# alanross/AlvaAR

Measured on NVIDIA H100. Metric: frames_per_sec_720p_1000orb_20kf_ba, higher is better.
Workload: dtype u8/f64

## Files before the change

alvaar_b200/csrc/ba.cu:

```cuda
#include "alva_common.cuh"
#include "../../include/alva_b200.h"
#include <math.h>
#include <float.h>
#include <string.h>

namespace {

constexpr int NMAX = 128;
constexpr int LIN_THREADS = 128;
constexpr int NBMAX = NMAX / 6;
constexpr int MAXKEYS = NBMAX * (NBMAX + 1) / 2;
constexpr int BS_THREADS = 128;

struct BaState {
    double radius, decrease_factor, x_cost, cand_cost, xnorm, gmax, model_change;
    double se_min, se_cur, se_ref, se_cand, se_acc_ref, se_acc_cand;
    double initial_cost, push_cost;
    int reuse_diagonal, invalid_steps, iteration, last_success, n_success, n_iter, term, done;
    int relin, step_ok, ncols, chol_ok;
    int use_gather, nb, nbad, has_last;
    int skipped, pad0;
};

struct BaProblem {
    const double* calib;
    double* poses;
    const uint8_t* pose_const;
    double* invd;
    const int32_t* anch_kf;
    const double* anch_uv;
    const int32_t* obs_kf;
    const int32_t* obs_lm;
    const double* obs_uv;
    double *res, *Ja, *Jd;
    double *wp;
    double *nf, *gf, *scf, *diagf, *Df;
    double *ne, *ge, *sce, *diage, *De;
    double *ete, *etb, *wa, *ye;
    double *S, *rhs, *yf;
    double *cand_poses, *cand_invd;
    double *cost_part;
    int32_t *pose_col;
    int32_t *lm_start, *lm_obs;
    double* Wt;
    double* mc_part;
    double* ga_part;
    int32_t* ga_ticket;
    int32_t *obs_col, *anch_col;
    int32_t *pstart;
    uint32_t *plist;
    int32_t *blk_start;
    int32_t *blk_off;
    uint64_t *pairs;
    const int32_t* obs_lm_in;
    int32_t* obs_lm_w;
    int32_t* flags;
    double *last_poses, *last_invd;
    BaState* st;
};

struct BaDims { int nkf, nlm, nobs, nblk; double huber; int max_iter; int nlm_pad; int ecap; int nbs; int pass; };

__device__ __forceinline__ void quat_to_R(const double* q, double* R) {
    const double n = sqrt(q[0] * q[0] + q[1] * q[1] + q[2] * q[2] + q[3] * q[3]);
    const double x = q[0] / n, y = q[1] / n, z = q[2] / n, w = q[3] / n;
    const double tx = 2 * x, ty = 2 * y, tz = 2 * z;
    const double twx = tx * w, twy = ty * w, twz = tz * w, txx = tx * x, txy = ty * x, txz = tz * x;
    const double tyy = ty * y, tyz = tz * y, tzz = tz * z;
    R[0] = 1 - (tyy + tzz); R[1] = txy - twz;       R[2] = txz + twy;
    R[3] = txy + twz;       R[4] = 1 - (txx + tzz); R[5] = tyz - twx;
    R[6] = txz - twy;       R[7] = tyz + twx;       R[8] = 1 - (txx + tyy);
}

__device__ void se3_plus(const double* x, const double* delta, double* out) {
    const double* ups = delta;
    const double* om = delta + 3;
    const double theta_sq = om[0] * om[0] + om[1] * om[1] + om[2] * om[2];
    const double eps = 1e-10;
    double theta, imag, real;
    if (theta_sq < eps * eps) {
        theta = 0;
        const double t4 = theta_sq * theta_sq;
        imag = 0.5 - (1.0 / 48.0) * theta_sq + (1.0 / 3840.0) * t4;
        real = 1.0 - (1.0 / 8.0) * theta_sq + (1.0 / 384.0) * t4;
    } else {
        theta = sqrt(theta_sq);
        const double half = 0.5 * theta;
        imag = sin(half) / theta;
        real = cos(half);
    }
    const double dq[4] = {imag * om[0], imag * om[1], imag * om[2], real};
    double Rd[9];
    quat_to_R(dq, Rd);
    const double O[9] = {0, -om[2], om[1], om[2], 0, -om[0], -om[1], om[0], 0};
    double V[9];
    if (theta < eps) {
        for (int i = 0; i < 9; i++) V[i] = Rd[i];
    } else {
        const double a = (1 - cos(theta)) / theta_sq, b = (theta - sin(theta)) / (theta_sq * theta);
        for (int i = 0; i < 3; i++)
            for (int j = 0; j < 3; j++) {
                double o2 = 0;
                for (int k = 0; k < 3; k++) o2 += O[3 * i + k] * O[3 * k + j];
                V[3 * i + j] = (i == j ? 1.0 : 0.0) + a * O[3 * i + j] + b * o2;
            }
    }
    for (int i = 0; i < 3; i++)
        out[i] = V[3 * i] * ups[0] + V[3 * i + 1] * ups[1] + V[3 * i + 2] * ups[2] + Rd[3 * i] * x[0] + Rd[3 * i + 1] * x[1] +
                 Rd[3 * i + 2] * x[2];
    const double qn = sqrt(x[3] * x[3] + x[4] * x[4] + x[5] * x[5] + x[6] * x[6]);
    const double bx = x[3] / qn, by = x[4] / qn, bz = x[5] / qn, bw = x[6] / qn;
    const double ax = dq[0], ay = dq[1], az = dq[2], aw = dq[3];
    double q[4] = {aw * bx + ax * bw + ay * bz - az * by, aw * by + ay * bw + az * bx - ax * bz,
                   aw * bz + az * bw + ax * by - ay * bx, aw * bw - ax * bx - ay * by - az * bz};
    const double n = sqrt(q[0] * q[0] + q[1] * q[1] + q[2] * q[2] + q[3] * q[3]);
    for (int i = 0; i < 4; i++) out[3 + i] = q[i] / n;
}

__device__ __forceinline__ bool ba_evaluate(const double* calib, const double* anch, const double* pose, double invd, double u,
                                            double v, double ua, double va, double* res, double* Ja, double* Jp, double* Jd) {
    const double fx = calib[0], fy = calib[1], cx = calib[2], cy = calib[3];
    double Rwa[9], Rwc[9];
    quat_to_R(anch + 3, Rwa);
    quat_to_R(pose + 3, Rwc);
    const double zanch = 1.0 / invd;
    const double ap[3] = {zanch * (ua - cx) / fx, zanch * (va - cy) / fy, zanch};
    double Ra[3], wpt[3];
    for (int i = 0; i < 3; i++) {
        Ra[i] = Rwa[3 * i] * ap[0] + Rwa[3 * i + 1] * ap[1] + Rwa[3 * i + 2] * ap[2];
        wpt[i] = Ra[i] + anch[i];
    }
    const double d[3] = {wpt[0] - pose[0], wpt[1] - pose[1], wpt[2] - pose[2]};
    double cp[3];
    for (int i = 0; i < 3; i++) cp[i] = Rwc[i] * d[0] + Rwc[3 + i] * d[1] + Rwc[6 + i] * d[2];
    const double iz = 1.0 / cp[2];
// ... 151 lines not shown
            if (P.obs_col[o] >= 0) { key = P.obs_col[o] / 6; val = ((uint32_t)l << 8) | (uint32_t)(i - P.lm_start[l] + 1); }
        }
    };
    int maxobs = 0;
    for (int l = tid; l < D.nlm; l += NT) maxobs = max(maxobs, P.lm_start[l + 1] - P.lm_start[l]);
    for (int t = tid; t < nitems; t += NT) {
        int key; uint32_t val;
        item(t, key, val);
        if (key >= 0) atomicAdd(&pl_base[key + 1], 1);
    }
    __syncthreads();
    if (tid == 0) {
        P.pstart[0] = 0;
        for (int k = 0; k < NBMAX; k++) { P.pstart[k + 1] = pl_base[k + 1]; pl_base[k + 1] += pl_base[k]; }
    }
    __syncthreads();
    for (int t0 = 0; t0 < nitems; t0 += NT) {
        for (int i = tid; i < 32 * (NBMAX + 1); i += NT) (&wcount[0][0])[i] = 0;
        __syncthreads();
        int key; uint32_t val;
        item(t0 + tid, key, val);
        const uint32_t m = __match_any_sync(0xffffffffu, key);
        const int rank = __popc(m & ((1u << lane) - 1));
        if (key >= 0 && rank == 0) wcount[warp][key] = __popc(m);
        __syncthreads();
        if (tid < NBMAX) {
            int acc = 0;
            for (int wv = 0; wv < 32; wv++) { const int c = wcount[wv][tid]; wcount[wv][tid] = acc; acc += c; }
            scan_s[tid] = acc;
        }
        __syncthreads();
        if (key >= 0) P.plist[pl_base[key] + run[key] + wcount[warp][key] + rank] = val;
        __syncthreads();
        if (tid < NBMAX) run[tid] += scan_s[tid];
        __syncthreads();
    }
    maxobs = max(maxobs, __shfl_xor_sync(0xffffffffu, maxobs, 16)); maxobs = max(maxobs, __shfl_xor_sync(0xffffffffu, maxobs, 8));
    maxobs = max(maxobs, __shfl_xor_sync(0xffffffffu, maxobs, 4)); maxobs = max(maxobs, __shfl_xor_sync(0xffffffffu, maxobs, 2));
    maxobs = max(maxobs, __shfl_xor_sync(0xffffffffu, maxobs, 1));
    if (lane == 0) scan_s[warp] = maxobs;
    __syncthreads();
    if (tid == 0) {
        int mo = 0;
        for (int i = 0; i < NT / 32; i++) mo = max(mo, scan_s[i]);
        P.st->use_gather = (mo < 255 && D.nlm < 65536 && D.nobs < 65535) ? 1 : 0;
    }
}

template <bool FULL>
__device__ __forceinline__ double lin_obs(const BaProblem& P, const BaDims& D, int o, int l, const double* poses, double invd_l) {
    const int ka = P.anch_kf[l], kp = P.obs_kf[o];
    double r[2], Ja[12], Jp[12], Jd[2];
    ba_evaluate(P.calib, poses + 7 * ka, poses + 7 * kp, invd_l, P.obs_uv[2 * o], P.obs_uv[2 * o + 1], P.anch_uv[2 * l],
                P.anch_uv[2 * l + 1], r, FULL ? Ja : nullptr, Jp, Jd);
    double rho0, rho1;
    huber(r[0] * r[0] + r[1] * r[1], D.huber, rho0, rho1);
    if (FULL) {
        const double sc = sqrt(rho1);
        r[0] *= sc; r[1] *= sc;
        P.res[2 * o] = r[0]; P.res[2 * o + 1] = r[1];
        Jd[0] *= sc; Jd[1] *= sc;
        P.Jd[2 * o] = Jd[0]; P.Jd[2 * o + 1] = Jd[1];
#pragma unroll
        for (int i = 0; i < 12; i++) { Ja[i] *= sc; P.Ja[12 * o + i] = Ja[i]; }
    }
    return 0.5 * rho0;
}

template <bool FULL>
__global__ void __launch_bounds__(LIN_THREADS, 7) ba_linearize_kernel(const BaProblem* __restrict__ probs, BaDims D) {
    const BaProblem P = probs[blockIdx.y];
    __shared__ double red[LIN_THREADS];
    const BaState& st = *P.st;
    const bool active = FULL ? (st.relin && !st.done) : !st.done;
    if (!active) return;
    const int o = blockIdx.x * LIN_THREADS + threadIdx.x;
    double cost = 0;
    const int l = o < D.nobs ? P.obs_lm[o] : -1;
    if (l >= 0) cost = lin_obs<FULL>(P, D, o, l, FULL ? P.poses : P.cand_poses, (FULL ? P.invd : P.cand_invd)[l]);
    const double tot = block_sum<LIN_THREADS>(cost, red);
    if (threadIdx.x == 0) P.cost_part[blockIdx.x] = tot;
}

__device__ __forceinline__ void stats_landmark(const BaProblem& P, int l) {
    double ne = 0, ge = 0;
    for (int i = P.lm_start[l]; i < P.lm_start[l + 1]; i++) {
        const int o = P.lm_obs[i];
        const double d0 = P.Jd[2 * o], d1 = P.Jd[2 * o + 1];
        ne += d0 * d0 + d1 * d1;
        ge += d0 * P.res[2 * o] + d1 * P.res[2 * o + 1];
    }
    P.ne[l] = ne;
    P.ge[l] = ge;
}
__device__ __forceinline__ void stats_pose_partial(const BaProblem& P, int b, int gt, double* v) {
    int eb = 0;
    for (int i = 0; i < b; i++) eb += P.pstart[i + 1];
    const int ee = eb + P.pstart[b + 1];
#pragma unroll
    for (int i = 0; i < 12; i++) v[i] = 0;
    for (int idx = eb + gt; idx < ee; idx += BS_THREADS) {
        const uint32_t en = P.plist[idx];
        const int l = en >> 8, su = en & 0xff;
        const int ob = P.lm_start[l];
        if (su) {
            const int o = P.lm_obs[ob + su - 1];
            const double r0 = P.res[2 * o], r1 = P.res[2 * o + 1];
#pragma unroll
            for (int c = 0; c < 6; c++) {
                const double j0 = -P.Ja[12 * o + c], j1 = -P.Ja[12 * o + 6 + c];
                v[c] += j0 * j0 + j1 * j1;
                v[6 + c] += j0 * r0 + j1 * r1;
            }
        } else {
            for (int i = ob; i < P.lm_start[l + 1]; i++) {
                const int o = P.lm_obs[i];
                const double r0 = P.res[2 * o], r1 = P.res[2 * o + 1];
#pragma unroll
                for (int c = 0; c < 6; c++) {
                    const double j0 = P.Ja[12 * o + c], j1 = P.Ja[12 * o + 6 + c];
                    v[c] += j0 * j0 + j1 * j1;
                    v[6 + c] += j0 * r0 + j1 * r1;
                }
            }
        }
    }
}

__global__ void __launch_bounds__(BS_THREADS) ba_stats_kernel(const BaProblem* __restrict__ probs, BaDims D) {
    const BaProblem P = probs[blockIdx.y];
    const BaState& st = *P.st;
    if (st.done || !st.relin) return;
    __shared__ double part[4][12];
    if ((int)blockIdx.x < D.nbs) {
        const int l = blockIdx.x * BS_THREADS + threadIdx.x;
        if (l >= D.nlm) return;
        stats_landmark(P, l);
        return;
    }
    const int b = blockIdx.x - D.nbs;
    if (b >= st.ncols / 6) return;
    const int lane = threadIdx.x & 31, warp = threadIdx.x >> 5;
    double v[12];
    stats_pose_partial(P, b, threadIdx.x, v);
#pragma unroll
    for (int i = 0; i < 12; i++) {
#pragma unroll
        for (int off = 16; off; off >>= 1) v[i] += __shfl_xor_sync(0xffffffffu, v[i], off);
        if (lane == 0) part[warp][i] = v[i];
    }
    __syncthreads();
    if (threadIdx.x < 12) {
        const double t = part[0][threadIdx.x] + part[1][threadIdx.x] + part[2][threadIdx.x] + part[3][threadIdx.x];
        if (threadIdx.x < 6) P.nf[6 * b + threadIdx.x] = t;
        else P.gf[6 * b + threadIdx.x - 6] = t;
    }
}

template <int MODE>
__global__ void __launch_bounds__(32) ba_pairs_kernel(const BaProblem* __restrict__ probs, BaDims D) {
    const BaProblem P = probs[blockIdx.y];
    BaState& st = *P.st;
    const int nb = st.ncols / 6, bi = blockIdx.x, lane = threadIdx.x;
    if (!st.use_gather) return;
    __shared__ int cnt[NBMAX];
    __shared__ int boff[NBMAX];
    if (bi >= nb) {
        if (MODE == 0) for (int bj = lane; bj < NBMAX; bj += 32) P.blk_start[bi * NBMAX + bj + 1] = 0;
        return;
    }
    int base_row = 0;
    if (MODE == 1) {
        int sum = 0;
        for (int i = lane; i < bi * NBMAX; i += 32) sum += P.blk_start[i + 1];
#pragma unroll
        for (int off = 16; off; off >>= 1) sum += __shfl_xor_sync(0xffffffffu, sum, off);
        base_row = sum;
    }
    if (lane < NBMAX) cnt[lane] = 0;
    if (lane == 0) {
        int run = base_row;
        for (int bj = 0; bj < NBMAX; bj++) {
            boff[bj] = run;
            if (MODE == 1) { P.blk_off[bi * NBMAX + bj] = run; run += P.blk_start[bi * NBMAX + bj + 1]; }
        }
    }
    __syncwarp();
    int eb = 0;
    for (int i = 0; i < bi; i++) eb += P.pstart[i + 1];
    const int ee = eb + P.pstart[bi + 1];
    for (int c0 = eb; c0 < ee; c0 += 32) {
        const int idx = c0 + lane;
        const bool live = idx < ee;
        const uint32_t en = live ? P.plist[idx] : 0u;
        const int l = en >> 8, su = en & 0xff;
        const int ob = live ? P.lm_start[l] : 0, ns = live ? P.lm_start[l + 1] - ob : -1;
        int cv0 = -1, cv1 = -1, cv2 = -1, cv3 = -1, o1 = -1, o2 = -1, o3 = -1, ou = 0xffff;
        if (live) {
            cv0 = P.anch_col[l];
            o1 = ns >= 1 ? P.lm_obs[ob] : -1; o2 = ns >= 2 ? P.lm_obs[ob + 1] : -1; o3 = ns >= 3 ? P.lm_obs[ob + 2] : -1;
            if (o1 >= 0) cv1 = P.obs_col[o1];
            if (o2 >= 0) cv2 = P.obs_col[o2];
            if (o3 >= 0) cv3 = P.obs_col[o3];
            if (MODE == 1 && su) ou = su == 1 ? o1 : su == 2 ? o2 : su == 3 ? o3 : P.lm_obs[ob + su - 1];
        }
        for (int sv = 0; sv <= 255; sv++) {
            if (!__any_sync(0xffffffffu, live && sv <= ns)) break;
            int bjv = -1, bjv_ov = 0xffff;
            if (live && sv <= ns) {
                const int ov = sv == 0 ? 0xffff : sv == 1 ? o1 : sv == 2 ? o2 : sv == 3 ? o3 : P.lm_obs[ob + sv - 1];
                bjv_ov = ov;
                const int cv = sv == 0 ? cv0 : sv == 1 ? cv1 : sv == 2 ? cv2 : sv == 3 ? cv3 : P.obs_col[ov];
                if (cv >= 0) { const int bj = cv / 6; if (bj > bi || (bj == bi && sv >= su)) bjv = bj; }
                if (MODE == 0 && cv >= 0 && cv / 6 == bi && sv > su) st.use_gather = 0;
            }
            const uint32_t m = __match_any_sync(0xffffffffu, bjv);
            if (bjv >= 0) {
                const int rank = __popc(m & ((1u << lane) - 1));
                const int old = cnt[bjv];
                if (MODE == 1) {
                    const int pos = boff[bjv] + old + rank;
                    if (pos < D.ecap)
                        P.pairs[pos] = ((uint64_t)l << 48) | ((uint64_t)su << 40) | ((uint64_t)sv << 32) | ((uint64_t)(ou & 0xffff) << 16) |
                                       (uint64_t)(bjv_ov & 0xffff);
                }
                __syncwarp(m);
                if (rank == 0) cnt[bjv] = old + __popc(m);
            }
            __syncwarp();
        }
    }
    if (MODE == 0) {
        if (lane < NBMAX) P.blk_start[bi * NBMAX + lane + 1] = cnt[lane];
    } else if (bi == nb - 1 && lane == 0) {
        int total = base_row;
        for (int bj = 0; bj < NBMAX; bj++) total += cnt[bj];
        if (total > D.ecap) st.use_gather = 0;
    }
}

constexpr int CT_THREADS = 1024;
__device__ void ba_pre_body(const BaProblem& P, const BaDims& D) {
    BaState& st = *P.st;
    __shared__ double red[34];
    __shared__ int go;
    const int tid = threadIdx.x, NT = blockDim.x;
    const int n = st.ncols;
    if (st.done) return;
    if (st.relin) {
        double c = 0;
        for (int i = tid; i < D.nblk; i += NT) c += P.cost_part[i];
        const double x_cost = block_sum_dyn(c, red);
        double xn = 0;
        for (int k = tid; k < D.nkf; k += NT)
            if (P.pose_col[k] >= 0) for (int i = 0; i < 7; i++) xn += P.poses[7 * k + i] * P.poses[7 * k + i];
        for (int l = tid; l < D.nlm; l += NT)
            if (P.lm_start[l + 1] > P.lm_start[l]) xn += P.invd[l] * P.invd[l];
        xn = block_sum_dyn(xn, red);
        double gm = 0;
        for (int k = tid; k < D.nkf; k += NT) {
            const int c0 = P.pose_col[k];
            if (c0 < 0) continue;
            double dlt[6], out[7];
            for (int i = 0; i < 6; i++) dlt[i] = -P.gf[c0 + i];
            se3_plus(P.poses + 7 * k, dlt, out);
            for (int i = 0; i < 7; i++) gm = fmax(gm, fabs(P.poses[7 * k + i] - out[i]));
        }
        for (int l = tid; l < D.nlm; l += NT)
            if (P.lm_start[l + 1] > P.lm_start[l]) gm = fmax(gm, fabs(P.ge[l]));
        gm = block_max_dyn(gm, red);
        if (st.iteration == 0) {
            for (int i = tid; i < n; i += NT) P.scf[i] = 1.0 / (1.0 + sqrt(P.nf[i]));
            for (int l = tid; l < D.nlm; l += NT) P.sce[l] = 1.0 / (1.0 + sqrt(P.ne[l]));
        }
        __syncthreads();
        if (tid == 0) {
            st.x_cost = x_cost; st.xnorm = sqrt(xn); st.gmax = gm; st.push_cost = x_cost;
            if (st.iteration == 0) {
                st.initial_cost = x_cost;
                st.se_min = st.se_cur = st.se_ref = st.se_cand = x_cost;
            }
            st.relin = 0;
        }
    }
    __syncthreads();
    if (tid == 0) {
        if (st.last_success) st.n_success++;
        st.n_iter++;
        int cont = 1;
        if (st.iteration >= D.max_iter) { st.term = 1; cont = 0; }
        else if (st.last_success && st.gmax <= 1e-10) { st.term = 0; cont = 0; }
        else if (st.radius <= 1e-32) { st.term = 0; cont = 0; }
        if (!cont) st.done = 1;
        else { st.iteration++; st.last_success = 0; }
        go = cont;
    }
    __syncthreads();
    if (!go) return;
    const bool reuse = st.reuse_diagonal;
    const double radius = st.radius;
    __syncthreads();
    for (int i = tid; i < n; i += NT) {
        if (!reuse) P.diagf[i] = fmin(fmax(P.nf[i] * P.scf[i] * P.scf[i], 1e-6), 1e32);
        P.Df[i] = sqrt(P.diagf[i] / radius);
    }
    for (int l = tid; l < D.nlm; l += NT) {
        if (!reuse) P.diage[l] = fmin(fmax(P.ne[l] * P.sce[l] * P.sce[l], 1e-6), 1e32);
        P.De[l] = sqrt(P.diage[l] / radius);
    }
    for (int i = tid; i < NMAX * NMAX; i += NT) P.S[i] = 0;
    for (int i = tid; i < NMAX; i += NT) P.rhs[i] = 0;
    __syncthreads();
    for (int i = tid; i < n; i += NT) P.S[i * NMAX + i] = P.Df[i] * P.Df[i];
    if (tid == 0) st.reuse_diagonal = 1;
}

__global__ void __launch_bounds__(CT_THREADS) ba_pre_kernel(const BaProblem* __restrict__ probs, BaDims D) {
    const BaProblem P = probs[blockIdx.x];
    ba_pre_body(P, D);
}

template <bool DENSE>
__device__ void schur_landmark(const BaProblem& P, const BaDims& D, int l) {
    if (DENSE) {
        double* row = P.Wt + (size_t)l * NMAX;
        for (int i = 0; i < NMAX; i++) row[i] = 0.0;
    }
    if (l >= D.nlm) return;
    const int b = P.lm_start[l], e = P.lm_start[l + 1];
    if (e == b) return;
    const int ca = P.pose_col[P.anch_kf[l]];
    const double sce = P.sce[l];
    double ete = P.De[l] * P.De[l], etb = 0, wa[6] = {0, 0, 0, 0, 0, 0};
    double sca[6];
    for (int c = 0; c < 6; c++) sca[c] = ca >= 0 ? P.scf[ca + c] : 0.0;
    double Saa[36];
    for (int i = 0; i < 36; i++) Saa[i] = 0;
    double rha[6] = {0, 0, 0, 0, 0, 0};
    for (int i = b; i < e; i++) {
        const int o = P.lm_obs[i];
        const int cp = P.pose_col[P.obs_kf[o]];
        const double e0 = P.Jd[2 * o] * sce, e1 = P.Jd[2 * o + 1] * sce;
        const double r0 = P.res[2 * o], r1 = P.res[2 * o + 1];
        ete += e0 * e0 + e1 * e1;
        etb += e0 * r0 + e1 * r1;
        double Fa[12], Fp[12];
        for (int c = 0; c < 6; c++) {
            Fa[c] = P.Ja[12 * o + c] * sca[c]; Fa[6 + c] = P.Ja[12 * o + 6 + c] * sca[c];
            const double s = cp >= 0 ? P.scf[cp + c] : 0.0;
            Fp[c] = -P.Ja[12 * o + c] * s; Fp[6 + c] = -P.Ja[12 * o + 6 + c] * s;
        }
        for (int c = 0; c < 6; c++) {
            wa[c] += e0 * Fa[c] + e1 * Fa[6 + c];
            P.wp[6 * o + c] = e0 * Fp[c] + e1 * Fp[6 + c];
            rha[c] += Fa[c] * r0 + Fa[6 + c] * r1;
        }
        if (ca >= 0)
            for (int a = 0; a < 6; a++)
                for (int c = 0; c < 6; c++) Saa[6 * a + c] += Fa[a] * Fa[c] + Fa[6 + a] * Fa[6 + c];
        if (cp >= 0) {
            for (int a = 0; a < 6; a++) {
                atomicAdd(&P.rhs[cp + a], Fp[a] * r0 + Fp[6 + a] * r1);
                for (int c = 0; c < 6; c++) {
                    atomicAdd(&P.S[(cp + a) * NMAX + cp + c], Fp[a] * Fp[c] + Fp[6 + a] * Fp[6 + c]);
                    if (ca >= 0) {
                        const double x = Fa[a] * Fp[c] + Fa[6 + a] * Fp[6 + c];
                        atomicAdd(&P.S[(ca + a) * NMAX + cp + c], x);
                        atomicAdd(&P.S[(cp + c) * NMAX + ca + a], x);
                    }
                }
            }
        }
    }
    const double inv = 1.0 / ete;
    P.ete[l] = ete;
    P.etb[l] = etb;
    for (int c = 0; c < 6; c++) P.wa[6 * l + c] = wa[c];
    if (ca >= 0)
        for (int a = 0; a < 6; a++) {
            atomicAdd(&P.rhs[ca + a], rha[a] - wa[a] * inv * etb);
            for (int c = 0; c < 6; c++)
                atomicAdd(&P.S[(ca + a) * NMAX + ca + c], DENSE ? Saa[6 * a + c] : Saa[6 * a + c] - wa[a] * inv * wa[c]);
        }
    if (DENSE) {
        const double rs = sqrt(inv);
        double* row = P.Wt + (size_t)l * NMAX;
        if (ca >= 0) for (int c = 0; c < 6; c++) row[ca + c] += wa[c] * rs;
        for (int i = b; i < e; i++) {
            const int oi = P.lm_obs[i];
            const int ci = P.pose_col[P.obs_kf[oi]];
            if (ci < 0) continue;
// ... 10 lines not shown
        if (ci < 0) continue;
        double wi[6];
        for (int c = 0; c < 6; c++) wi[c] = P.wp[6 * oi + c];
        for (int a = 0; a < 6; a++) atomicAdd(&P.rhs[ci + a], -wi[a] * inv * etb);
        if (ca >= 0)
            for (int a = 0; a < 6; a++)
                for (int c = 0; c < 6; c++) {
                    const double x = -wa[a] * inv * wi[c];
                    atomicAdd(&P.S[(ca + a) * NMAX + ci + c], x);
                    atomicAdd(&P.S[(ci + c) * NMAX + ca + a], x);
                }
        for (int j = b; j < e; j++) {
            const int oj = P.lm_obs[j];
            const int cj = P.pose_col[P.obs_kf[oj]];
            if (cj < 0) continue;
            for (int a = 0; a < 6; a++)
                for (int c = 0; c < 6; c++) atomicAdd(&P.S[(ci + a) * NMAX + cj + c], -wi[a] * inv * P.wp[6 * oj + c]);
        }
    }
}

template <bool DENSE>
__global__ void __launch_bounds__(128) ba_schur_kernel(const BaProblem* __restrict__ probs, BaDims D) {
    const BaProblem P = probs[blockIdx.y];
    if (P.st->done) return;
    if (!DENSE && P.st->use_gather) return;
    const int l = blockIdx.x * 128 + threadIdx.x;
    if (l >= D.nlm_pad) return;
    schur_landmark<DENSE>(P, D, l);
}

__device__ __forceinline__ void dmma_m8n8k4(double& c0, double& c1, double a, double b) {
    asm volatile("mma.sync.aligned.m8n8k4.row.col.f64.f64.f64.f64 {%0, %1}, {%2}, {%3}, {%0, %1};"
                 : "+d"(c0), "+d"(c1)
                 : "d"(a), "d"(b));
}

constexpr int SYRK_KSPLIT = 8;

__global__ void __launch_bounds__(128) ba_syrk_dmma_kernel(const BaProblem* __restrict__ probs, BaDims D) {
    const BaProblem P = probs[blockIdx.z];
    if (P.st->done) return;
    __shared__ double part[4][32][33];
    const int lane = threadIdx.x & 31, warp = threadIdx.x >> 5;
    const int bi = blockIdx.x >> 2, bj = blockIdx.x & 3;
    const int i0 = bi * 32, j0 = bj * 32;
    const int n = P.st->ncols;
    if (i0 >= n || j0 >= n) return;
    const int ksteps = D.nlm_pad / 4;
    const int per = (ksteps + SYRK_KSPLIT - 1) / SYRK_KSPLIT;
    const int kb = blockIdx.y * per, ke = min(ksteps, kb + per);
    double acc[4][4][2];
#pragma unroll
    for (int a = 0; a < 4; a++)
#pragma unroll
        for (int b = 0; b < 4; b++) acc[a][b][0] = acc[a][b][1] = 0.0;
    const int kr = lane & 3, cc = lane >> 2;
    for (int ks = kb + warp; ks < ke; ks += 4) {
        const double* row = P.Wt + (size_t)(4 * ks + kr) * NMAX;
        double av[4], bv[4];
#pragma unroll
        for (int t = 0; t < 4; t++) { av[t] = __ldg(row + i0 + 8 * t + cc); bv[t] = __ldg(row + j0 + 8 * t + cc); }
#pragma unroll
        for (int a = 0; a < 4; a++)
#pragma unroll
            for (int b = 0; b < 4; b++) dmma_m8n8k4(acc[a][b][0], acc[a][b][1], av[a], bv[b]);
    }
#pragma unroll
    for (int a = 0; a < 4; a++)
#pragma unroll
        for (int b = 0; b < 4; b++) {
            part[warp][8 * a + cc][8 * b + 2 * kr] = acc[a][b][0];
            part[warp][8 * a + cc][8 * b + 2 * kr + 1] = acc[a][b][1];
        }
    __syncthreads();
    for (int t = threadIdx.x; t < 32 * 32; t += 128) {
        const int r = t >> 5, c = t & 31;
        const double v = part[0][r][c] + part[1][r][c] + part[2][r][c] + part[3][r][c];
        if (v != 0.0) atomicAdd(&P.S[(i0 + r) * NMAX + j0 + c], -v);
    }
}


__device__ __forceinline__ void lm_landmark(const BaProblem& P, int l) {
    const int b = P.lm_start[l], e = P.lm_start[l + 1];
    if (e == b) return;
    const int ca = P.pose_col[P.anch_kf[l]];
    const double sce = P.sce[l];
    double ete = P.De[l] * P.De[l], etb = 0, wa[6] = {0, 0, 0, 0, 0, 0};
    for (int i = b; i < e; i++) {
        const int o = P.lm_obs[i];
        const int cp = P.pose_col[P.obs_kf[o]];
        const double e0 = P.Jd[2 * o] * sce, e1 = P.Jd[2 * o + 1] * sce;
        ete += e0 * e0 + e1 * e1;
        etb += e0 * P.res[2 * o] + e1 * P.res[2 * o + 1];
        for (int c = 0; c < 6; c++) {
            if (ca >= 0) wa[c] += (e0 * P.Ja[12 * o + c] + e1 * P.Ja[12 * o + 6 + c]) * P.scf[ca + c];
            P.wp[6 * o + c] = cp >= 0 ? (e0 * -P.Ja[12 * o + c] + e1 * -P.Ja[12 * o + 6 + c]) * P.scf[cp + c] : 0.0;
        }
    }
    P.ete[l] = ete;
    P.etb[l] = etb;
    for (int c = 0; c < 6; c++) P.wa[6 * l + c] = wa[c];
}
__global__ void __launch_bounds__(128) ba_lm_kernel(const BaProblem* __restrict__ probs, BaDims D) {
    const BaProblem P = probs[blockIdx.y];
    if (P.st->done) return;
    const int l = blockIdx.x * 128 + threadIdx.x;
    if (P.st->use_gather) { if (l < D.nlm) lm_landmark(P, l); }
    else if (l < D.nlm) schur_landmark<false>(P, D, l);
}

template <bool TRANSPOSE>
__device__ __forceinline__ void gather_entry(const BaProblem& P, uint64_t en, const double* sci, const double* scj, double* acc,
                                             double* rh) {
    const int l = (int)(en >> 48), su = (int)(en >> 40) & 0xff, sv = (int)(en >> 32) & 0xff;
    const double inv = 1.0 / P.ete[l], etb = P.etb[l];
    const int ou = su ? (int)(en >> 16) & 0xffff : -1, ov = sv ? (int)en & 0xffff : -1;
    double wu[6], wv[6];
#pragma unroll
    for (int c = 0; c < 6; c++) {
        wu[c] = (su ? P.wp[6 * ou + c] : P.wa[6 * l + c]) * inv;
        wv[c] = sv ? P.wp[6 * ov + c] : P.wa[6 * l + c];
    }
#define ACC(a, c) acc[TRANSPOSE ? 6 * (c) + (a) : 6 * (a) + (c)]
#pragma unroll
    for (int a = 0; a < 6; a++)
#pragma unroll
        for (int c = 0; c < 6; c++) ACC(a, c) -= wu[a] * wv[c];
    if (su == 0 && sv == 0) {
        const int ob = P.lm_start[l], oe = P.lm_start[l + 1];
        for (int i = ob; i < oe; i++) {
            const int o = P.lm_obs[i];
            double F0[6], F1[6];
#pragma unroll
            for (int c = 0; c < 6; c++) { F0[c] = P.Ja[12 * o + c] * sci[c]; F1[c] = P.Ja[12 * o + 6 + c] * sci[c]; }
            const double r0 = P.res[2 * o], r1 = P.res[2 * o + 1];
#pragma unroll
            for (int a = 0; a < 6; a++) {
                if (!TRANSPOSE) rh[a] += F0[a] * r0 + F1[a] * r1;
#pragma unroll
                for (int c = 0; c < 6; c++) ACC(a, c) += F0[a] * F0[c] + F1[a] * F1[c];
            }
        }
        if (!TRANSPOSE)
#pragma unroll
            for (int a = 0; a < 6; a++) rh[a] -= wu[a] * etb;
    } else if (su == sv) {
        double F0[6], F1[6];
#pragma unroll
        for (int c = 0; c < 6; c++) { F0[c] = -P.Ja[12 * ou + c] * sci[c]; F1[c] = -P.Ja[12 * ou + 6 + c] * sci[c]; }
        const double r0 = P.res[2 * ou], r1 = P.res[2 * ou + 1];
#pragma unroll
        for (int a = 0; a < 6; a++) {
            if (!TRANSPOSE) rh[a] += F0[a] * r0 + F1[a] * r1 - wu[a] * etb;
#pragma unroll
            for (int c = 0; c < 6; c++) ACC(a, c) += F0[a] * F0[c] + F1[a] * F1[c];
        }
    } else if (su == 0 || sv == 0) {
        const int o = su ? ou : ov;
        double A0[6], A1[6];
#pragma unroll
        for (int a = 0; a < 6; a++) {
            A0[a] = (su ? -P.Ja[12 * o + a] : P.Ja[12 * o + a]) * sci[a];
            A1[a] = (su ? -P.Ja[12 * o + 6 + a] : P.Ja[12 * o + 6 + a]) * sci[a];
        }
#pragma unroll
        for (int c = 0; c < 6; c++) {
            const double b0 = (sv ? -P.Ja[12 * o + c] : P.Ja[12 * o + c]) * scj[c];
            const double b1 = (sv ? -P.Ja[12 * o + 6 + c] : P.Ja[12 * o + 6 + c]) * scj[c];
#pragma unroll
            for (int a = 0; a < 6; a++) ACC(a, c) += A0[a] * b0 + A1[a] * b1;
        }
    }
#undef ACC
}

constexpr int GA_THREADS = 64, GA_SPLIT = 8;
constexpr int GA_GRID = NBMAX * GA_SPLIT + (MAXKEYS - NBMAX);
__global__ void __launch_bounds__(GA_THREADS, 8) ba_gather_kernel(const BaProblem* __restrict__ probs, BaDims D) {
    const BaProblem P = probs[blockIdx.y];
    const BaState& st = *P.st;
    if (st.done || !st.use_gather) return;
    int bi, bj, part = 0, nparts = 1;
    if ((int)blockIdx.x < NBMAX * GA_SPLIT) { bi = bj = blockIdx.x / GA_SPLIT; part = blockIdx.x % GA_SPLIT; nparts = GA_SPLIT; }
    else {
        int rem = blockIdx.x - NBMAX * GA_SPLIT;
        bi = 0;
        while (bi < NBMAX - 1 && rem >= NBMAX - 1 - bi) { rem -= NBMAX - 1 - bi; bi++; }
        bj = bi + 1 + rem;
    }
    if (bi >= st.nb || bj >= st.nb) return;
// ... 332 lines not shown
__global__ void ba_linearize_dump_kernel(const double* calib, const double* poses, const double* invd, const int32_t* anch_kf,
                                         const double* anch_uv, const int32_t* obs_kf, const int32_t* obs_lm,
                                         const double* obs_uv, int nobs, double hub, double* res, double* Ja, double* Jp,
                                         double* Jd, double* cost) {
    const int o = blockIdx.x * blockDim.x + threadIdx.x;
    if (o >= nobs) return;
    const int l = obs_lm[o];
    double r[2] = {0, 0}, A[12], Pp[12], Dd[2];
    for (int i = 0; i < 12; i++) A[i] = Pp[i] = 0;
    Dd[0] = Dd[1] = 0;
    double c = 0;
    if (l >= 0) {
        ba_evaluate(calib, poses + 7 * anch_kf[l], poses + 7 * obs_kf[o], invd[l], obs_uv[2 * o], obs_uv[2 * o + 1],
                    anch_uv[2 * l], anch_uv[2 * l + 1], r, A, Pp, Dd);
        double rho0, rho1;
        huber(r[0] * r[0] + r[1] * r[1], hub, rho0, rho1);
        c = 0.5 * rho0;
        const double sc = sqrt(rho1);
        r[0] *= sc; r[1] *= sc; Dd[0] *= sc; Dd[1] *= sc;
        for (int i = 0; i < 12; i++) { A[i] *= sc; Pp[i] *= sc; }
    }
    res[2 * o] = r[0]; res[2 * o + 1] = r[1]; Jd[2 * o] = Dd[0]; Jd[2 * o + 1] = Dd[1];
    for (int i = 0; i < 12; i++) { Ja[12 * o + i] = A[i]; Jp[12 * o + i] = Pp[i]; }
    cost[o] = c;
}

__global__ void ba_local_init_kernel(const BaProblem* __restrict__ probs, BaDims D) {
    const BaProblem P = probs[blockIdx.y];
    const int o = blockIdx.x * blockDim.x + threadIdx.x;
    if (o < D.nobs) { P.obs_lm_w[o] = P.obs_lm_in[o]; P.flags[o] = 0; }
    if (o == 0) { P.st->nbad = 0; P.st->has_last = 0; P.st->skipped = 0; }
}

template <int MARK>
__global__ void __launch_bounds__(LIN_THREADS) ba_flag_kernel(const BaProblem* __restrict__ probs, BaDims D, double chi2_thr) {
    const BaProblem P = probs[blockIdx.y];
    BaState& st = *P.st;
    if (MARK == 2 && st.skipped) return;
    const int o = blockIdx.x * LIN_THREADS + threadIdx.x;
    const int l = o < D.nobs ? P.obs_lm_w[o] : -1;
    if (l < 0) return;
    const double* poses = st.has_last ? P.last_poses : P.poses;
    const double* invd = st.has_last ? P.last_invd : P.invd;
    double r[2];
    const bool front = ba_evaluate(P.calib, poses + 7 * P.anch_kf[l], poses + 7 * P.obs_kf[o], invd[l], P.obs_uv[2 * o],
                                   P.obs_uv[2 * o + 1], P.anch_uv[2 * l], P.anch_uv[2 * l + 1], r, nullptr, nullptr, nullptr);
    if (r[0] * r[0] + r[1] * r[1] > chi2_thr || !front) {
        P.flags[o] = MARK;
        if (MARK == 1) { P.obs_lm_w[o] = -1; atomicAdd(&st.nbad, 1); }
    }
}

__global__ void ba_summary_local_kernel(const BaProblem* __restrict__ probs, double* __restrict__ summary, int second) {
    const BaState& st = *probs[blockIdx.x].st;
    if (threadIdx.x == 0) {
        double* s = summary + 10 * blockIdx.x + 5 * second;
        if (second && st.skipped) { s[0] = s[1] = s[2] = s[3] = s[4] = 0; return; }
        s[0] = st.initial_cost; s[1] = st.x_cost; s[2] = st.n_success; s[3] = st.n_iter; s[4] = st.term;
    }
}

__global__ void ba_summary_kernel(const BaProblem* __restrict__ probs, double* __restrict__ summary) {
    const BaState& st = *probs[blockIdx.x].st;
    if (threadIdx.x == 0) {
        double* s = summary + 8 * blockIdx.x;
        s[0] = st.initial_cost; s[1] = st.x_cost; s[2] = st.n_success; s[3] = st.n_iter; s[4] = st.term;
        s[5] = st.ncols; s[6] = st.radius; s[7] = st.iteration;
    }
}

size_t align_up(size_t v, size_t a) { return (v + a - 1) / a * a; }

}

static int g_ba_dense_schur = 0;
static int g_ba_ctl_threads = CT_THREADS;

static size_t ba_ws_bytes(int nkf, int nlm, int nobs, int nblk) {
    size_t d = 0;
    if (g_ba_dense_schur) d += (size_t)((nlm + 3) / 4 * 4) * NMAX;
    d += (size_t)nobs * (2 + 12 + 2 + 6);
    d += 5 * (size_t)NMAX;
    d += 5 * (size_t)nlm;
    d += (size_t)nlm * (1 + 1 + 6 + 1);
    d += (size_t)NMAX * NMAX + 2 * NMAX;
    d += (size_t)nkf * 7 + nlm;
    d += (size_t)nblk;
    d += (size_t)((nlm + BS_THREADS - 1) / BS_THREADS);
    d += (size_t)NBMAX * GA_SPLIT * 42;
    size_t bytes = d * sizeof(double);
    bytes += align_up((size_t)nkf * 4, 8) + align_up((size_t)(nlm + 1) * 4, 8) + align_up((size_t)nobs * 4, 8);
    bytes += align_up((size_t)nobs * 4, 8) + align_up((size_t)nlm * 4, 8);
    bytes += align_up((size_t)(NBMAX + 1) * 4, 8) + align_up(((size_t)nobs + (size_t)nlm) * 4, 8);
    bytes += 2 * align_up((size_t)(NBMAX * NBMAX + 1) * 4, 8) + align_up((size_t)(8 * (size_t)nobs + 2 * (size_t)nlm) * 8, 8);
    bytes += align_up((size_t)NBMAX * 4, 8);
    bytes += align_up(sizeof(BaState), 8);
    return align_up(bytes, 256);
}

static int ba_prepare(alva_ctx* ctx, int nprob, int nkf, int nlm, int nobs, const double* calib, double* poses,
                      const uint8_t* pose_const, double* invd, const int32_t* anch_kf, const double* anch_uv,
                      const int32_t* obs_kf, const int32_t* obs_lm, const double* obs_uv, int32_t* flags,
                      const BaProblem** dp_out, BaDims* D_out) {
    const bool local = flags != nullptr;
    const int nblk = (nobs + LIN_THREADS - 1) / LIN_THREADS;
    const size_t per_local = align_up((size_t)nobs * 4, 8) + (7 * (size_t)nkf + (size_t)nlm) * sizeof(double);
    const size_t per = align_up(ba_ws_bytes(nkf, nlm, nobs, nblk) + (local ? per_local : 0), 256);
    const size_t tab = align_up(sizeof(BaProblem) * nprob, 256);
    if (tab + per * nprob > ctx->ba_ws_bytes) {
        if (ctx->ba_ws) { ALVA_CUDA(cudaStreamSynchronize(ctx->stream)); ALVA_CUDA(cudaFree(ctx->ba_ws)); ctx->ba_ws = nullptr; ctx->ba_ws_bytes = 0; }
        ALVA_CUDA(cudaMalloc(&ctx->ba_ws, tab + per * nprob));
        ctx->ba_ws_bytes = tab + per * nprob;
        ctx->ba_table_key = 0;
    }
    uint8_t* ws = (uint8_t*)ctx->ba_ws;
    uint64_t key = 1469598103934665603ull;
    auto mix = [&](uint64_t v) { key = (key ^ v) * 1099511628211ull; };
    mix((uint64_t)(uintptr_t)ws); mix(nprob); mix(nkf); mix(nlm); mix(nobs); mix((uint64_t)g_ba_dense_schur);
    mix((uint64_t)(uintptr_t)calib); mix((uint64_t)(uintptr_t)poses); mix((uint64_t)(uintptr_t)pose_const); mix((uint64_t)(uintptr_t)invd);
    mix((uint64_t)(uintptr_t)anch_kf); mix((uint64_t)(uintptr_t)anch_uv); mix((uint64_t)(uintptr_t)obs_kf);
    mix((uint64_t)(uintptr_t)obs_lm); mix((uint64_t)(uintptr_t)obs_uv); mix((uint64_t)(uintptr_t)flags);
    if (key != ctx->ba_table_key) {
        std::string hostbuf(sizeof(BaProblem) * nprob, '\0');
        BaProblem* hp = reinterpret_cast<BaProblem*>(&hostbuf[0]);
        for (int p = 0; p < nprob; p++) {
            BaProblem& P = hp[p];
            P.calib = calib + 4 * (size_t)p; P.poses = poses + 7 * (size_t)nkf * p; P.pose_const = pose_const + (size_t)nkf * p;
            P.invd = invd + (size_t)nlm * p; P.anch_kf = anch_kf + (size_t)nlm * p; P.anch_uv = anch_uv + 2 * (size_t)nlm * p;
            P.obs_kf = obs_kf + (size_t)nobs * p; P.obs_lm = obs_lm + (size_t)nobs * p; P.obs_uv = obs_uv + 2 * (size_t)nobs * p;
            double* d = reinterpret_cast<double*>(ws + tab + per * p);
            auto take = [&](size_t n) { double* r = d; d += n; return r; };
            P.res = take(2 * (size_t)nobs); P.Ja = take(12 * (size_t)nobs); P.Jd = take(2 * (size_t)nobs);
            P.wp = take(6 * (size_t)nobs);
            P.nf = take(NMAX); P.gf = take(NMAX); P.scf = take(NMAX); P.diagf = take(NMAX); P.Df = take(NMAX);
            P.ne = take(nlm); P.ge = take(nlm); P.sce = take(nlm); P.diage = take(nlm); P.De = take(nlm);
            P.ete = take(nlm); P.etb = take(nlm); P.wa = take(6 * (size_t)nlm); P.ye = take(nlm);
            P.S = take((size_t)NMAX * NMAX); P.rhs = take(NMAX); P.yf = take(NMAX);
            P.cand_poses = take(7 * (size_t)nkf); P.cand_invd = take(nlm); P.cost_part = take(nblk);
            P.Wt = g_ba_dense_schur ? take((size_t)((nlm + 3) / 4 * 4) * NMAX) : nullptr;
            P.mc_part = take((size_t)((nlm + BS_THREADS - 1) / BS_THREADS));
            P.ga_part = take((size_t)NBMAX * GA_SPLIT * 42);
            P.last_poses = local ? take(7 * (size_t)nkf) : nullptr;
            P.last_invd = local ? take(nlm) : nullptr;
            uint8_t* b = reinterpret_cast<uint8_t*>(d);
            P.pose_col = reinterpret_cast<int32_t*>(b); b += align_up((size_t)nkf * 4, 8);
            P.lm_start = reinterpret_cast<int32_t*>(b); b += align_up((size_t)(nlm + 1) * 4, 8);
            P.lm_obs = reinterpret_cast<int32_t*>(b); b += align_up((size_t)nobs * 4, 8);
            P.obs_col = reinterpret_cast<int32_t*>(b); b += align_up((size_t)nobs * 4, 8);
            P.anch_col = reinterpret_cast<int32_t*>(b); b += align_up((size_t)nlm * 4, 8);
            P.pstart = reinterpret_cast<int32_t*>(b); b += align_up((size_t)(NBMAX + 1) * 4, 8);
            P.plist = reinterpret_cast<uint32_t*>(b); b += align_up(((size_t)nobs + (size_t)nlm) * 4, 8);
            P.blk_start = reinterpret_cast<int32_t*>(b); b += align_up((size_t)(NBMAX * NBMAX + 1) * 4, 8);
            P.blk_off = reinterpret_cast<int32_t*>(b); b += align_up((size_t)(NBMAX * NBMAX + 1) * 4, 8);
            P.pairs = reinterpret_cast<uint64_t*>(b); b += align_up((size_t)(8 * (size_t)nobs + 2 * (size_t)nlm) * 8, 8);
            P.ga_ticket = reinterpret_cast<int32_t*>(b); b += align_up((size_t)NBMAX * 4, 8);
            P.obs_lm_in = nullptr; P.obs_lm_w = nullptr; P.flags = nullptr;
            if (local) {
                P.obs_lm_in = P.obs_lm;
                P.obs_lm_w = reinterpret_cast<int32_t*>(b); b += align_up((size_t)nobs * 4, 8);
                P.obs_lm = P.obs_lm_w;
                P.flags = flags + (size_t)nobs * p;
            }
            P.st = reinterpret_cast<BaState*>(b);
        }
        ALVA_CUDA(cudaMemcpyAsync(ws, hp, sizeof(BaProblem) * nprob, cudaMemcpyHostToDevice, ctx->stream));
        ALVA_CUDA(cudaStreamSynchronize(ctx->stream));
        ctx->ba_table_key = key;
    }
    *dp_out = reinterpret_cast<const BaProblem*>(ws);
    *D_out = BaDims{nkf, nlm, nobs, nblk, 0.0, 0, (nlm + 3) / 4 * 4, 8 * nobs + 2 * nlm, (nlm + BS_THREADS - 1) / BS_THREADS, 0};
    return 0;
}

static int ba_run_solve(alva_ctx* ctx, const BaProblem* dp, const BaDims& D, int nprob) {
    const bool dense = g_ba_dense_schur != 0;
    const size_t chol_smem = ((size_t)NMAX * (NMAX + 1) + NMAX) * sizeof(double);
    ALVA_CUDA(cudaFuncSetAttribute(ba_chol_kernel, cudaFuncAttributeMaxDynamicSharedMemorySize, (int)chol_smem));
    ba_setup_kernel<<<nprob, SETUP_THREADS, 0, ctx->stream>>>(dp, D);
    ALVA_LAUNCH_CHECK(ctx);
    const dim3 lin_grid(D.nblk, nprob), schur_grid((D.nlm_pad + 127) / 128, nprob), syrk_grid(16, SYRK_KSPLIT, nprob);
    const dim3 key_grid(GA_GRID, nprob), bs_grid(D.nbs, nprob), stats_grid(D.nbs + NBMAX, nprob);
    bool forked = false;
    if (!dense) {
        const dim3 pr_grid(NBMAX, nprob);
        cudaStream_t ps = ctx->stream;
        if (ctx->aux_stream && cudaEventRecord(ctx->aux_fork, ctx->stream) == cudaSuccess &&
            cudaStreamWaitEvent(ctx->aux_stream, ctx->aux_fork, 0) == cudaSuccess) { ps = ctx->aux_stream; forked = true; }
        ba_pairs_kernel<0><<<pr_grid, 32, 0, ps>>>(dp, D);
        ALVA_LAUNCH_CHECK(ctx);
        ba_pairs_kernel<1><<<pr_grid, 32, 0, ps>>>(dp, D);
        ALVA_LAUNCH_CHECK(ctx);
        if (forked) ALVA_CUDA(cudaEventRecord(ctx->aux_join, ps));
    }
    for (int it = 0; it <= D.max_iter; it++) {
        ba_linearize_kernel<true><<<lin_grid, LIN_THREADS, 0, ctx->stream>>>(dp, D);
        ALVA_LAUNCH_CHECK(ctx);
        ba_stats_kernel<<<stats_grid, BS_THREADS, 0, ctx->stream>>>(dp, D);
        ALVA_LAUNCH_CHECK(ctx);
        ba_pre_kernel<<<nprob, g_ba_ctl_threads, 0, ctx->stream>>>(dp, D);
        ALVA_LAUNCH_CHECK(ctx);
        if (it == D.max_iter) {
            if (forked) { ALVA_CUDA(cudaStreamWaitEvent(ctx->stream, ctx->aux_join, 0)); forked = false; }
            break;
        }
        if (dense) {
            ba_schur_kernel<true><<<schur_grid, 128, 0, ctx->stream>>>(dp, D);
            ALVA_LAUNCH_CHECK(ctx);
            ba_syrk_dmma_kernel<<<syrk_grid, 128, 0, ctx->stream>>>(dp, D);
            ALVA_LAUNCH_CHECK(ctx);
        } else {
            if (forked) { ALVA_CUDA(cudaStreamWaitEvent(ctx->stream, ctx->aux_join, 0)); forked = false; }
            ba_lm_kernel<<<schur_grid, 128, 0, ctx->stream>>>(dp, D);
            ALVA_LAUNCH_CHECK(ctx);
            ba_gather_kernel<<<key_grid, GA_THREADS, 0, ctx->stream>>>(dp, D);
            ALVA_LAUNCH_CHECK(ctx);
        }
        ba_chol_kernel<<<nprob, CH_THREADS, chol_smem, ctx->stream>>>(dp, D);
        ALVA_LAUNCH_CHECK(ctx);
        ba_backsub_kernel<<<bs_grid, BS_THREADS, 0, ctx->stream>>>(dp, D);
        ALVA_LAUNCH_CHECK(ctx);
        ba_linearize_kernel<false><<<lin_grid, LIN_THREADS, 0, ctx->stream>>>(dp, D);
        ALVA_LAUNCH_CHECK(ctx);
        ba_post_kernel<<<nprob, g_ba_ctl_threads, 0, ctx->stream>>>(dp, D);
        ALVA_LAUNCH_CHECK(ctx);
    }
    return 0;
}

static bool ba_args_ok(alva_ctx* ctx, int nprob, int nkf, int nlm, int nobs, const void* calib, const void* poses,
                       const void* pose_const, const void* invd, const void* anch_kf, const void* anch_uv, const void* obs_kf,
                       const void* obs_lm, const void* obs_uv, int max_iter) {
    return ctx && nprob >= 1 && nkf >= 1 && nkf <= 256 && nlm >= 1 && nobs >= 1 && calib && poses && pose_const && invd &&
           anch_kf && anch_uv && obs_kf && obs_lm && obs_uv && max_iter >= 0;
}

extern "C" int alva_k_ba_solve(alva_ctx* ctx, int nprob, int nkf, int nlm, int nobs, const double* calib, double* poses,
                               const uint8_t* pose_const, double* invd, const int32_t* anch_kf, const double* anch_uv,
                               const int32_t* obs_kf, const int32_t* obs_lm, const double* obs_uv, double huber_delta,
                               int max_iter, double* summary) { AlvaDeviceGuard guard__(ctx);
    if (!ba_args_ok(ctx, nprob, nkf, nlm, nobs, calib, poses, pose_const, invd, anch_kf, anch_uv, obs_kf, obs_lm, obs_uv, max_iter)) {
        alva_set_error("alva_k_ba_solve: bad argument (need 1 <= nkf <= 256)");
        return ALVA_E_INVALID;
    }
    const BaProblem* dp;
    BaDims D;
    if (int e = ba_prepare(ctx, nprob, nkf, nlm, nobs, calib, poses, pose_const, invd, anch_kf, anch_uv, obs_kf, obs_lm, obs_uv,
                           nullptr, &dp, &D))
        return e;
    D.huber = huber_delta; D.max_iter = max_iter;
    if (int e = ba_run_solve(ctx, dp, D, nprob)) return e;
    if (summary) {
        ba_summary_kernel<<<nprob, 32, 0, ctx->stream>>>(dp, summary);
        ALVA_LAUNCH_CHECK(ctx);
    }
    return 0;
}

extern "C" int alva_k_ba_local(alva_ctx* ctx, int nprob, int nkf, int nlm, int nobs, const double* calib, double* poses,
                               const uint8_t* pose_const, double* invd, const int32_t* anch_kf, const double* anch_uv,
                               const int32_t* obs_kf, const int32_t* obs_lm, const double* obs_uv, double huber_delta,
                               double chi2_thr, int max_iter, int32_t* flags, double* summary) { AlvaDeviceGuard guard__(ctx);
    if (!ba_args_ok(ctx, nprob, nkf, nlm, nobs, calib, poses, pose_const, invd, anch_kf, anch_uv, obs_kf, obs_lm, obs_uv, max_iter) ||
        !flags) {
        alva_set_error("alva_k_ba_local: bad argument (need 1 <= nkf <= 256, flags != NULL)");
        return ALVA_E_INVALID;
    }
    const BaProblem* dp;
    BaDims D;
    if (int e = ba_prepare(ctx, nprob, nkf, nlm, nobs, calib, poses, pose_const, invd, anch_kf, anch_uv, obs_kf, obs_lm, obs_uv,
                           flags, &dp, &D))
        return e;
    D.huber = huber_delta; D.max_iter = max_iter;
    const dim3 obs_grid(D.nblk, nprob);
// ... 53 lines not shown
```

Before: 39100.

## Fuse landmark Schur terms into stats kernel and split pair building across warps

The per-landmark Schur quantities (se2, etb, wa, wp) are now computed inside the stats kernel while the Jd/res data is already loaded. The LM kernel then only rescales wa and wp by the pose scaling on the first solve iteration, and ete is assembled in the pre kernel from the damping term plus the cached se2. Separately, the pair-building kernel now runs 8 warps per block-row instead of one, with per-warp counts stored in a new wcnt buffer so the offsets stay deterministic. The fusion depends on the pose scaling scf being fixed after iteration 0 and on stats running before pre, so it adds coupling and extra workspace in exchange for fewer passes over the Jacobians.

```diff
diff --git a/alvaar_b200/csrc/ba.cu b/alvaar_b200/csrc/ba.cu
--- a/alvaar_b200/csrc/ba.cu
+++ b/alvaar_b200/csrc/ba.cu
@@ -37,6 +37,7 @@
     double *nf, *gf, *scf, *diagf, *Df;
     double *ne, *ge, *sce, *diage, *De;
     double *ete, *etb, *wa, *ye;
+    double *se2;
     double *S, *rhs, *yf;
     double *cand_poses, *cand_invd;
     double *cost_part;
@@ -51,6 +52,7 @@
     uint32_t *plist;
     int32_t *blk_start;
     int32_t *blk_off;
+    int32_t *wcnt;
     uint64_t *pairs;
     const int32_t* obs_lm_in;
     int32_t* obs_lm_w;
@@ -368,9 +370,10 @@
     if (threadIdx.x == 0) P.cost_part[blockIdx.x] = tot;
 }
 
-__device__ __forceinline__ void stats_landmark(const BaProblem& P, int l) {
+__device__ __forceinline__ void stats_landmark(const BaProblem& P, int l, bool first) {
+    const int b = P.lm_start[l], e = P.lm_start[l + 1];
     double ne = 0, ge = 0;
-    for (int i = P.lm_start[l]; i < P.lm_start[l + 1]; i++) {
+    for (int i = b; i < e; i++) {
         const int o = P.lm_obs[i];
         const double d0 = P.Jd[2 * o], d1 = P.Jd[2 * o + 1];
         ne += d0 * d0 + d1 * d1;
@@ -378,6 +381,27 @@
     }
     P.ne[l] = ne;
     P.ge[l] = ge;
+    double sce;
+    if (first) { sce = 1.0 / (1.0 + sqrt(ne)); P.sce[l] = sce; }
+    else sce = P.sce[l];
+    if (e == b) { P.se2[l] = 0; return; }
+    const int ca = P.pose_col[P.anch_kf[l]];
+    double se2 = 0, etb = 0, wa[6] = {0, 0, 0, 0, 0, 0};
+    for (int i = b; i < e; i++) {
+        const int o = P.lm_obs[i];
+        const int cp = P.pose_col[P.obs_kf[o]];
+        const double e0 = P.Jd[2 * o] * sce, e1 = P.Jd[2 * o + 1] * sce;
+        se2 += e0 * e0 + e1 * e1;
+        etb += e0 * P.res[2 * o] + e1 * P.res[2 * o + 1];
+        for (int c = 0; c < 6; c++) {
+            const double ja0 = P.Ja[12 * o + c], ja1 = P.Ja[12 * o + 6 + c];
+            if (ca >= 0) wa[c] += first ? e0 * ja0 + e1 * ja1 : (e0 * ja0 + e1 * ja1) * P.scf[ca + c];
+            P.wp[6 * o + c] = cp < 0 ? 0.0 : first ? e0 * -ja0 + e1 * -ja1 : (e0 * -ja0 + e1 * -ja1) * P.scf[cp + c];
+        }
+    }
+    P.se2[l] = se2;
+    P.etb[l] = etb;
+    for (int c = 0; c < 6; c++) P.wa[6 * l + c] = wa[c];
 }
 __device__ __forceinline__ void stats_pose_partial(const BaProblem& P, int b, int gt, double* v) {
     int eb = 0;
@@ -421,7 +445,7 @@
     if ((int)blockIdx.x < D.nbs) {
         const int l = blockIdx.x * BS_THREADS + threadIdx.x;
         if (l >= D.nlm) return;
-        stats_landmark(P, l);
+        stats_landmark(P, l, st.iteration == 0);
         return;
     }
     const int b = blockIdx.x - D.nbs;
@@ -443,18 +467,23 @@
     }
 }
 
+constexpr int PR_WARPS = 8;
 template <int MODE>
-__global__ void __launch_bounds__(32) ba_pairs_kernel(const BaProblem* __restrict__ probs, BaDims D) {
+__global__ void __launch_bounds__(32 * PR_WARPS) ba_pairs_kernel(const BaProblem* __restrict__ probs, BaDims D) {
     const BaProblem P = probs[blockIdx.y];
     BaState& st = *P.st;
-    const int nb = st.ncols / 6, bi = blockIdx.x, lane = threadIdx.x;
-    if (!st.use_gather) return;
-    __shared__ int cnt[NBMAX];
-    __shared__ int boff[NBMAX];
+    const int nb = st.ncols / 6, bi = blockIdx.x, lane = threadIdx.x & 31, warp = threadIdx.x >> 5;
+    __shared__ int go;
+    __shared__ int cnt[PR_WARPS][NBMAX];
+    __shared__ int boff[PR_WARPS][NBMAX];
+    if (threadIdx.x == 0) go = st.use_gather;
+    __syncthreads();
+    if (!go) return;
     if (bi >= nb) {
-        if (MODE == 0) for (int bj = lane; bj < NBMAX; bj += 32) P.blk_start[bi * NBMAX + bj + 1] = 0;
+        if (MODE == 0) for (int bj = threadIdx.x; bj < NBMAX; bj += blockDim.x) P.blk_start[bi * NBMAX + bj + 1] = 0;
         return;
     }
+    int* wc = P.wcnt + (size_t)bi * PR_WARPS * NBMAX;
     int base_row = 0;
     if (MODE == 1) {
         int sum = 0;
@@ -463,21 +492,26 @@
         for (int off = 16; off; off >>= 1) sum += __shfl_xor_sync(0xffffffffu, sum, off);
         base_row = sum;
     }
-    if (lane < NBMAX) cnt[lane] = 0;
-    if (lane == 0) {
+    if (lane < NBMAX) cnt[warp][lane] = 0;
+    if (MODE == 1 && lane == 0) {
         int run = base_row;
         for (int bj = 0; bj < NBMAX; bj++) {
-            boff[bj] = run;
-            if (MODE == 1) { P.blk_off[bi * NBMAX + bj] = run; run += P.blk_start[bi * NBMAX + bj + 1]; }
+            int before = 0;
+            for (int w = 0; w < warp; w++) before += wc[w * NBMAX + bj];
+            boff[warp][bj] = run + before;
+            if (warp == 0) P.blk_off[bi * NBMAX + bj] = run;
+            run += P.blk_start[bi * NBMAX + bj + 1];
         }
     }
     __syncwarp();
     int eb = 0;
     for (int i = 0; i < bi; i++) eb += P.pstart[i + 1];
     const int ee = eb + P.pstart[bi + 1];
-    for (int c0 = eb; c0 < ee; c0 += 32) {
+    const int nchunk = (ee - eb + 31) / 32, per = (nchunk + PR_WARPS - 1) / PR_WARPS;
+    const int cb = eb + 32 * min(nchunk, warp * per), ce = min(ee, eb + 32 * min(nchunk, (warp + 1) * per));
+    for (int c0 = cb; c0 < ce; c0 += 32) {
         const int idx = c0 + lane;
-        const bool live = idx < ee;
+        const bool live = idx < ce;
         const uint32_t en = live ? P.plist[idx] : 0u;
         const int l = en >> 8, su = en & 0xff;
         const int ob = live ? P.lm_start[l] : 0, ns = live ? P.lm_start[l + 1] - ob : -1;
@@ -503,24 +537,30 @@
             const uint32_t m = __match_any_sync(0xffffffffu, bjv);
             if (bjv >= 0) {
                 const int rank = __popc(m & ((1u << lane) - 1));
-                const int old = cnt[bjv];
+                const int old = cnt[warp][bjv];
                 if (MODE == 1) {
-                    const int pos = boff[bjv] + old + rank;
+                    const int pos = boff[warp][bjv] + old + rank;
                     if (pos < D.ecap)
                         P.pairs[pos] = ((uint64_t)l << 48) | ((uint64_t)su << 40) | ((uint64_t)sv << 32) | ((uint64_t)(ou & 0xffff) << 16) |
                                        (uint64_t)(bjv_ov & 0xffff);
                 }
                 __syncwarp(m);
-                if (rank == 0) cnt[bjv] = old + __popc(m);
+                if (rank == 0) cnt[warp][bjv] = old + __popc(m);
             }
             __syncwarp();
         }
     }
     if (MODE == 0) {
-        if (lane < NBMAX) P.blk_start[bi * NBMAX + lane + 1] = cnt[lane];
-    } else if (bi == nb - 1 && lane == 0) {
+        if (lane < NBMAX) wc[warp * NBMAX + lane] = cnt[warp][lane];
+        __syncthreads();
+        if (threadIdx.x < NBMAX) {
+            int t = 0;
+            for (int w = 0; w < PR_WARPS; w++) t += cnt[w][threadIdx.x];
+            P.blk_start[bi * NBMAX + threadIdx.x + 1] = t;
+        }
+    } else if (bi == nb - 1 && threadIdx.x == 0) {
         int total = base_row;
-        for (int bj = 0; bj < NBMAX; bj++) total += cnt[bj];
+        for (int bj = 0; bj < NBMAX; bj++) total += P.blk_start[bi * NBMAX + bj + 1];
         if (total > D.ecap) st.use_gather = 0;
     }
 }
@@ -555,10 +595,8 @@
         for (int l = tid; l < D.nlm; l += NT)
             if (P.lm_start[l + 1] > P.lm_start[l]) gm = fmax(gm, fabs(P.ge[l]));
         gm = block_max_dyn(gm, red);
-        if (st.iteration == 0) {
+        if (st.iteration == 0)
             for (int i = tid; i < n; i += NT) P.scf[i] = 1.0 / (1.0 + sqrt(P.nf[i]));
-            for (int l = tid; l < D.nlm; l += NT) P.sce[l] = 1.0 / (1.0 + sqrt(P.ne[l]));
-        }
         __syncthreads();
         if (tid == 0) {
             st.x_cost = x_cost; st.xnorm = sqrt(xn); st.gmax = gm; st.push_cost = x_cost;
@@ -592,7 +630,9 @@
     }
     for (int l = tid; l < D.nlm; l += NT) {
         if (!reuse) P.diage[l] = fmin(fmax(P.ne[l] * P.sce[l] * P.sce[l], 1e-6), 1e32);
-        P.De[l] = sqrt(P.diage[l] / radius);
+        const double De = sqrt(P.diage[l] / radius);
+        P.De[l] = De;
+        P.ete[l] = De * De + P.se2[l];
     }
     for (int i = tid; i < NMAX * NMAX; i += NT) P.S[i] = 0;
     for (int i = tid; i < NMAX; i += NT) P.rhs[i] = 0;
@@ -769,32 +809,22 @@
 }
 
 
-__device__ __forceinline__ void lm_landmark(const BaProblem& P, int l) {
+__device__ __forceinline__ void scale_landmark(const BaProblem& P, int l) {
     const int b = P.lm_start[l], e = P.lm_start[l + 1];
     if (e == b) return;
     const int ca = P.pose_col[P.anch_kf[l]];
-    const double sce = P.sce[l];
-    double ete = P.De[l] * P.De[l], etb = 0, wa[6] = {0, 0, 0, 0, 0, 0};
+    if (ca >= 0) for (int c = 0; c < 6; c++) P.wa[6 * l + c] *= P.scf[ca + c];
     for (int i = b; i < e; i++) {
         const int o = P.lm_obs[i];
         const int cp = P.pose_col[P.obs_kf[o]];
-        const double e0 = P.Jd[2 * o] * sce, e1 = P.Jd[2 * o + 1] * sce;
-        ete += e0 * e0 + e1 * e1;
-        etb += e0 * P.res[2 * o] + e1 * P.res[2 * o + 1];
-        for (int c = 0; c < 6; c++) {
-            if (ca >= 0) wa[c] += (e0 * P.Ja[12 * o + c] + e1 * P.Ja[12 * o + 6 + c]) * P.scf[ca + c];
-            P.wp[6 * o + c] = cp >= 0 ? (e0 * -P.Ja[12 * o + c] + e1 * -P.Ja[12 * o + 6 + c]) * P.scf[cp + c] : 0.0;
-        }
-    }
-    P.ete[l] = ete;
-    P.etb[l] = etb;
-    for (int c = 0; c < 6; c++) P.wa[6 * l + c] = wa[c];
+        if (cp >= 0) for (int c = 0; c < 6; c++) P.wp[6 * o + c] *= P.scf[cp + c];
+    }
 }
 __global__ void __launch_bounds__(128) ba_lm_kernel(const BaProblem* __restrict__ probs, BaDims D) {
     const BaProblem P = probs[blockIdx.y];
     if (P.st->done) return;
     const int l = blockIdx.x * 128 + threadIdx.x;
-    if (P.st->use_gather) { if (l < D.nlm) lm_landmark(P, l); }
+    if (P.st->use_gather) { if (l < D.nlm && P.st->iteration == 1) scale_landmark(P, l); }
     else if (l < D.nlm) schur_landmark<false>(P, D, l);
 }
 
@@ -1293,7 +1323,7 @@
     d += (size_t)nobs * (2 + 12 + 2 + 6);
     d += 5 * (size_t)NMAX;
     d += 5 * (size_t)nlm;
-    d += (size_t)nlm * (1 + 1 + 6 + 1);
+    d += (size_t)nlm * (1 + 1 + 6 + 1 + 1);
     d += (size_t)NMAX * NMAX + 2 * NMAX;
     d += (size_t)nkf * 7 + nlm;
     d += (size_t)nblk;
@@ -1305,6 +1335,7 @@
     bytes += align_up((size_t)(NBMAX + 1) * 4, 8) + align_up(((size_t)nobs + (size_t)nlm) * 4, 8);
     bytes += 2 * align_up((size_t)(NBMAX * NBMAX + 1) * 4, 8) + align_up((size_t)(8 * (size_t)nobs + 2 * (size_t)nlm) * 8, 8);
     bytes += align_up((size_t)NBMAX * 4, 8);
+    bytes += align_up((size_t)NBMAX * PR_WARPS * NBMAX * 4, 8);
     bytes += align_up(sizeof(BaState), 8);
     return align_up(bytes, 256);
 }
@@ -1345,7 +1376,7 @@
             P.wp = take(6 * (size_t)nobs);
             P.nf = take(NMAX); P.gf = take(NMAX); P.scf = take(NMAX); P.diagf = take(NMAX); P.Df = take(NMAX);
             P.ne = take(nlm); P.ge = take(nlm); P.sce = take(nlm); P.diage = take(nlm); P.De = take(nlm);
-            P.ete = take(nlm); P.etb = take(nlm); P.wa = take(6 * (size_t)nlm); P.ye = take(nlm);
+            P.ete = take(nlm); P.etb = take(nlm); P.wa = take(6 * (size_t)nlm); P.ye = take(nlm); P.se2 = take(nlm);
             P.S = take((size_t)NMAX * NMAX); P.rhs = take(NMAX); P.yf = take(NMAX);
             P.cand_poses = take(7 * (size_t)nkf); P.cand_invd = take(nlm); P.cost_part = take(nblk);
             P.Wt = g_ba_dense_schur ? take((size_t)((nlm + 3) / 4 * 4) * NMAX) : nullptr;
@@ -1365,6 +1396,7 @@
             P.blk_off = reinterpret_cast<int32_t*>(b); b += align_up((size_t)(NBMAX * NBMAX + 1) * 4, 8);
             P.pairs = reinterpret_cast<uint64_t*>(b); b += align_up((size_t)(8 * (size_t)nobs + 2 * (size_t)nlm) * 8, 8);
             P.ga_ticket = reinterpret_cast<int32_t*>(b); b += align_up((size_t)NBMAX * 4, 8);
+            P.wcnt = reinterpret_cast<int32_t*>(b); b += align_up((size_t)NBMAX * PR_WARPS * NBMAX * 4, 8);
             P.obs_lm_in = nullptr; P.obs_lm_w = nullptr; P.flags = nullptr;
             if (local) {
                 P.obs_lm_in = P.obs_lm;
@@ -1397,9 +1429,9 @@
         cudaStream_t ps = ctx->stream;
         if (ctx->aux_stream && cudaEventRecord(ctx->aux_fork, ctx->stream) == cudaSuccess &&
             cudaStreamWaitEvent(ctx->aux_stream, ctx->aux_fork, 0) == cudaSuccess) { ps = ctx->aux_stream; forked = true; }
-        ba_pairs_kernel<0><<<pr_grid, 32, 0, ps>>>(dp, D);
+        ba_pairs_kernel<0><<<pr_grid, 32 * PR_WARPS, 0, ps>>>(dp, D);
         ALVA_LAUNCH_CHECK(ctx);
-        ba_pairs_kernel<1><<<pr_grid, 32, 0, ps>>>(dp, D);
+        ba_pairs_kernel<1><<<pr_grid, 32 * PR_WARPS, 0, ps>>>(dp, D);
         ALVA_LAUNCH_CHECK(ctx);
         if (forked) ALVA_CUDA(cudaEventRecord(ctx->aux_join, ps));
     }
```

New measurement: 40240 (median of 6 runs). +2.9%, better.
